# KumarRobotics/AllocNet

Hardware: AMD Instinct MI355X
Metric: MINCO trajectories solved/sec (8-seg min-snap) (higher is better)
Workload: dtype f64; 1 GPU; configs[1] problem (8-segment order-4 MINCO, random-walk waypoints, energy-only, PVA boundary c=3) at saturating batch 1048576/GPU; batch_per_gpu=1048576, row_stride_ld=1049152, pieces=8, order=4, global_batch=1048576, parallelism=dp1, ranks_seen=1, allgather_bytes_per_rank=0, allgather_every=1

## Files before the change

allocnet_amd/csrc/qp_ipm.h:

```cpp
#pragma once
#include <hip/hip_runtime.h>
#include <stdint.h>

#include <type_traits>

#include "minco_core.h"
#include "wave_ops.h"
#include "qp_admm.h"
#include "workspace_constants.h"
#include "qp_control_points.h"

namespace anet {

struct IpmArgs {
  const double *state;
  const double *T;
  const double *hpolys;
  double *sl, *lam;
  double *coeffs;
  double *obj;
  int *status, *iters;
  double *res;
  double *gradT;
  const double *grad_z;
  double *vjpT;
  int64_t B;
  int N, R, M;
  double vmax, amax, m34, tol;
  int max_iter;
  double tol_accept;
  double tol_tenth;
  int twist_min_pieces;
  const int *order;
  int it_stop, resume;
  double *cont;
  const double *tab;
#ifdef ANET_IPM_PROF
  long long *prof;
#endif
};
#ifdef ANET_IPM_PROF
#define IPM_TICK(slot)                                                          \
  do {                                                                          \
    __syncthreads();                                                            \
    if (a.prof && blockIdx.x == 0 && threadIdx.x == 0) {                        \
      const long long now_ = __builtin_readcyclecounter();                      \
      a.prof[slot] += now_ - prof_t_;                                           \
      prof_t_ = now_;                                                           \
    }                                                                           \
  } while (0)
#else
#define IPM_TICK(slot) do {} while (0)
#endif

struct IpmCorridorRow {
  double c0, c1, c2;
  static constexpr int dsel = 0;
  __device__ __forceinline__ double dot(const double (&v)[3]) const { return c0 * v[0] + c1 * v[1] + c2 * v[2]; }
  __device__ __forceinline__ void axpy(double t, double *g) const { g[0] += t * c0; g[1] += t * c1; g[2] += t * c2; }
  __device__ __forceinline__ void weights(double w, double *A) const {
    A[0] += w * c0 * c0; A[1] += w * c0 * c1; A[2] += w * c0 * c2;
    A[3] += w * c1 * c1; A[4] += w * c1 * c2; A[5] += w * c2 * c2;
  }
};
struct IpmBoxRow {
  int ax, dsel;
  double sgn;
  __device__ __forceinline__ double dot(const double (&v)[3]) const { return sgn * v[ax]; }
  __device__ __forceinline__ void axpy(double t, double *g) const { g[ax] += sgn * t; }
  __device__ __forceinline__ void weights(double w, double *A) const { A[3 + dsel * 3 + ax] += w; }
};

__host__ __device__ constexpr int ipm_ht_stride(int D) { return 3 * D + 1; }
constexpr int kIpmRecord = 31;

template <int S>
inline size_t qp_ipm_lds_bytes(int N, int R, int M) {
  constexpr int D = 2 * S, NB = 3 * D, BK = 3 * S;
  const size_t NS = (size_t)N * R;
  return sizeof(double) * ((size_t)(N + 1) * BK * 5 + (size_t)(N + 1) * BK * BK + (size_t)N * BK * BK + 3 * (size_t)N * NB +
                           (size_t)R * ipm_ht_stride(D) + 2 * D * D + (size_t)N * D + NS * kIpmRecord + (size_t)N * M * 4 + 2 * N + 32);
}

template <int S>
__global__ void __launch_bounds__(256) k_qp_ipm_tables(double *out, int R, double m34, int control_points) {
  constexpr int D = 2 * S, HS = ipm_ht_stride(D);
  const int tid = threadIdx.x, nt = blockDim.x;
  __shared__ double E[2 * D * D], Hm[D * D];
  double *Hobj = out + D * D, *ht = out + 2 * D * D;
  if (tid == 0) {
    constexpr int W = 2 * D;
    for (int r = 0; r < D; ++r)
      for (int col = 0; col < D; ++col) {
        const int d = r % S, k = D - 1 - col;
        double v = 0.0;
        if (k >= d) v = (r < S) ? (k == d ? fallf(k, d) : 0.0) : fallf(k, d);
        E[r * W + col] = v;
        E[r * W + D + col] = (r == col) ? 1.0 : 0.0;
      }
    for (int c = 0; c < D; ++c) {
      int pv = c;
      for (int r = c + 1; r < D; ++r)
        if (fabs(E[r * W + c]) > fabs(E[pv * W + c])) pv = r;
      for (int k = 0; k < W; ++k) { const double t = E[c * W + k]; E[c * W + k] = E[pv * W + k]; E[pv * W + k] = t; }
      const double ip = 1.0 / E[c * W + c];
      for (int k = 0; k < W; ++k) E[c * W + k] *= ip;
      for (int r = 0; r < D; ++r)
        if (r != c) {
          const double f = E[r * W + c];
          if (f != 0.0)
            for (int k = 0; k < W; ++k) E[r * W + k] -= f * E[c * W + k];
        }
    }
    for (int r = 0; r < D; ++r)
      for (int c = 0; c < D; ++c) Hm[r * D + c] = E[r * W + D + c];
  }
  __syncthreads();
  if (control_points) {
    const int K = R / D;
    for (int e = tid; e < K * 3 * D; e += nt) {
      const int q = e / (3 * D), d = (e / D) % 3, m = e % D;
      double c[D], beta[D];
      for (int k = 0; k < D; ++k) c[k] = Hm[(D - 1 - k) * D + m];
      qp_control_values<D>(c, d, q, K, beta);
      for (int r = 0; r < D; ++r) ht[(size_t)(q * D + r) * HS + d * D + m] = beta[r];
    }
  }
  const int n_sampled = control_points ? 0 : R * 3 * D;
  for (int e = tid; e < n_sampled; e += nt) {
    const int j = e / (3 * D), d = (e / D) % 3, m = e % D;
    const double tau = (double)j / (double)R;
    double v = 0.0;
    for (int col = 0; col < D; ++col) {
      const int k = D - 1 - col;
      if (k >= d) {
        double bv = fallf(k, d);
        for (int q = 0; q < k - d; ++q) bv *= tau;
        v += bv * Hm[col * D + m];
      }
    }
    ht[(size_t)j * HS + d * D + m] = v;
  }
  for (int e = tid; e < D * D; e += nt) {
    const int m = e / D, m2 = e % D;
    double v = 0.0;
    for (int c1 = 0; c1 < S; ++c1)
      for (int c2 = 0; c2 < S; ++c2) v += Hm[c1 * D + m] * qblk1<S>(c1, c2, m34) * Hm[c2 * D + m2];
    Hobj[e] = v;
  }
  for (int e = tid; e < D * D; e += nt) out[e] = Hm[e];
}

template <int S, int MINB = 1, bool FUSE = (MINB == 1)>
__global__ void __launch_bounds__(256, MINB) k_qp_ipm(IpmArgs a) {
  constexpr int D = 2 * S, NB = 3 * D, BK = 3 * S;
  constexpr int HS = ipm_ht_stride(D), AS = kIpmRecord;
  const int N = a.N, R = a.R, M = a.M;
  const int NS = N * R, RPS = M + 12;
  const int64_t mtot = (int64_t)NS * RPS;
  const int64_t b = a.order ? (int64_t)a.order[blockIdx.x] : (int64_t)blockIdx.x;
  const int tid = threadIdx.x, nt = blockDim.x;
  const int NY = (N + 1) * BK;
  const bool resume = a.resume != 0;
  if ((uint64_t)b >= (uint64_t)a.B) return;
  if (resume && a.status[b] != 0) return;
  double *ct = a.cont ? a.cont + b * (int64_t)(NY + kIpmContScalars) : nullptr;

#ifdef ANET_IPM_PROF
  const long long prof_start_ = __builtin_readcyclecounter();
#endif
  extern __shared__ double lds[];
  double *yv = lds;
  double *dya = yv + NY;
  double *dyc = dya + NY;
  double *rhs = dyc + NY;
  double *Dg = rhs + NY;
  double *Of = Dg + (size_t)(N + 1) * BK * BK;
  double *uu = Of + (size_t)N * BK * BK;
  double *dua = uu + (size_t)N * NB;
  double *duc = dua + (size_t)N * NB;
  double *ht = duc + (size_t)N * NB;
  double *Hobj = ht + (size_t)R * HS;
  double *Hm = Hobj + D * D;
  double *sc = Hm + D * D;
  double *acc = sc + (size_t)N * D;
  double *hp_l = acc + (size_t)NS * AS;
  double *Tn = hp_l + (size_t)N * M * 4;
  double *red = Tn + N;
  double *qsv = red + 32;
  double *dinvd = qsv + N;

  const double *Tg = a.T + b * N;
  const double *hp = a.hpolys + b * (int64_t)N * M * 4;
  const double *st = a.state + b * 18;
  double *slg = a.sl + b * mtot, *lmg = a.lam + b * mtot;

  for (int e = tid; e < N * M * 4; e += nt) hp_l[e] = hp[e];
  for (int i = tid; i < N; i += nt) {
    Tn[i] = Tg[i];
    qsv[i] = pow(Tg[i], (double)(1 - 2 * S));
  }
  {
    const double *tb = a.tab;
    for (int e = tid; e < D * D; e += nt) {
      Hm[e] = tb[e];
      Hobj[e] = tb[D * D + e];
    }
    for (int e = tid; e < R * HS; e += nt) ht[e] = tb[2 * D * D + e];
  }
  __syncthreads();
  for (int e = tid; e < N * D; e += nt) {
    const int i = e / D, m = e % D;
    double v = 1.0;
    if (m >= S && i < N - 1) v = pow(Tn[i] / Tn[i + 1], (double)(m - S));
    sc[e] = v;
  }
  for (int e = tid; e < NY; e += nt) {
    const int k = e / BK, ax = (e / S) % 3, d = e % S;
    double v = 0.0;
    if (k == 0 && d < 3) v = st[ax * 3 + d] * pow(Tn[0], (double)d);
    else if (k == N && d < 3) v = st[9 + ax * 3 + d] * pow(Tn[N - 1], (double)d);
    else if (d == 0) {
      double tsum = 0.0, tk = 0.0;
      for (int i = 0; i < N; ++i) { tsum += Tn[i]; if (i < k) tk += Tn[i]; }
      const double f = tk / tsum;
      v = (1.0 - f) * st[ax * 3] + f * st[9 + ax * 3];
    }
    yv[e] = resume ? ct[e] : v;
    dya[e] = 0.0;
    dyc[e] = 0.0;
  }
  __syncthreads();
  auto uni = [](double v) {
    return __hiloint2double(__builtin_amdgcn_readfirstlane(__double2hiint(v)), __builtin_amdgcn_readfirstlane(__double2loint(v)));
  };
  auto pinned = [&](int k, int d) { return (k == 0 || k == N) && d < 3; };
  auto fresh_tid = [&]() {
    int t = tid;
    asm volatile("" : "+v"(t));
    return t;
  };
  auto to_u = [&](const double *y, double *u) {
    for (int e = fresh_tid(); e < N * NB; e += nt) {
      const int i = e / NB, ax = (e % NB) / D, m = e % D;
      u[e] = (m < S) ? y[i * BK + ax * S + m] : sc[i * D + m] * y[(i + 1) * BK + ax * S + (m - S)];
    }
  };
  to_u(yv, uu);
  __syncthreads();

  auto state_of = [&](const double *u, int i, int j, double (&s3)[3][3]) {
    const double *hj = ht + (size_t)j * HS, *ui = u + (size_t)i * NB;
#pragma unroll
    for (int d = 0; d < 3; ++d)
#pragma unroll
      for (int ax = 0; ax < 3; ++ax) {
        double v = 0.0;
        for (int m = 0; m < D; ++m) v += hj[d * D + m] * ui[ax * D + m];
        s3[d][ax] = v;
      }
  };
  auto for_rows = [&](int i, auto &&fn) {
    for (int q = 0; q < M; ++q) {
      const double *hq = hp_l + ((size_t)i * M + q) * 4;
      const double c0 = hq[0], c1 = hq[1], c2 = hq[2];
      if (c0 == 0.0 && c1 == 0.0 && c2 == 0.0) continue;
      fn(q, IpmCorridorRow{c0, c1, c2}, hq[3]);
    }
    const double hvv = a.vmax * Tn[i], hva = a.amax * Tn[i] * Tn[i];
#pragma unroll
    for (int qq = 0; qq < 12; ++qq) {
      const int axsel = qq / 4, w4 = qq % 4, dsel = 1 + (w4 & 1);
      const double sgn = (w4 < 2) ? 1.0 : -1.0;
      fn(M + qq, IpmBoxRow{axsel, dsel, sgn}, dsel == 1 ? hvv : hva);
    }
  };
  auto for_rows_sl = [&](int i, int smp, auto store_tag, auto &&fn) {
    constexpr bool STORE = decltype(store_tag)::value;
    double *sp = slg + smp, *lp = lmg + smp;
    constexpr int GC = (STORE && FUSE) ? 4 : 8, GB = (STORE && FUSE) ? 4 : 6;
    for (int q0 = 0; q0 < M; q0 += GC) {
      double sl[GC], lm[GC];
#pragma unroll
      for (int g = 0; g < GC; ++g) {
        const int q = q0 + g < M ? q0 + g : M - 1;
        sl[g] = sp[(int64_t)q * NS];
        lm[g] = lp[(int64_t)q * NS];
      }
#pragma unroll
      for (int g = 0; g < GC; ++g) {
        const int q = q0 + g;
        if (q >= M) break;
        const double *hq = hp_l + ((size_t)i * M + q) * 4;
        const double c0 = hq[0], c1 = hq[1], c2 = hq[2];
        if (c0 == 0.0 && c1 == 0.0 && c2 == 0.0) continue;
        fn(q, IpmCorridorRow{c0, c1, c2}, hq[3], sl[g], lm[g]);
        if (STORE) {
          sp[(int64_t)q * NS] = sl[g];
          lp[(int64_t)q * NS] = lm[g];
        }
      }
    }
    const double hvv = a.vmax * Tn[i], hva = a.amax * Tn[i] * Tn[i];
#pragma unroll
    for (int g0 = 0; g0 < 12; g0 += GB) {
      double sl[GB], lm[GB];
#pragma unroll
      for (int g = 0; g < GB; ++g) {
        sl[g] = sp[(int64_t)(M + g0 + g) * NS];
        lm[g] = lp[(int64_t)(M + g0 + g) * NS];
      }
#pragma unroll
      for (int g = 0; g < GB; ++g) {
        const int qq = g0 + g, axsel = qq / 4, w4 = qq % 4, dsel = 1 + (w4 & 1);
        const double sgn = (w4 < 2) ? 1.0 : -1.0;
        fn(M + qq, IpmBoxRow{axsel, dsel, sgn}, dsel == 1 ? hvv : hva, sl[g], lm[g]);
        if (STORE) {
          sp[(int64_t)(M + qq) * NS] = sl[g];
          lp[(int64_t)(M + qq) * NS] = lm[g];
        }
      }
    }
  };
  using RowsLoad = std::integral_constant<bool, false>;
  using RowsUpdate = std::integral_constant<bool, true>;
  auto sum_index = [](int slot) { return slot == 0 ? 0 : (slot == 4 ? 1 : (slot == 5 ? 2 : 3)); };
  auto block_reduce = [&](double v, int slot, bool is_min) {
    v = is_min ? wave_min_f64(v) : wave_sum<63>(v);
    if ((tid & 63) == 0) {
      if (is_min) atomic_max_pos(&red[slot], 1.0 / fmax(v, 1e-300));
      else red[16 + 4 * sum_index(slot) + (tid >> 6)] = v;
    }
  };
  auto red_sum = [&](int slot) {
    const double *p4 = red + 16 + 4 * sum_index(slot);
    return (p4[0] + p4[1]) + (p4[2] + p4[3]);
  };

#ifndef ANET_IPM_LAM0_SCALE
#define ANET_IPM_LAM0_SCALE 1e-6
#endif
  auto first_iterate = [&]() -> double {
  if (tid < 32) red[tid] = 0.0;
  __syncthreads();
  {
    double l_p = 0.0;
    for (int e = tid; e < NY; e += nt) {
      const int k = e / BK, ax = (e / S) % 3, d = e % S;
      if (pinned(k, d)) continue;
      double vp = 0.0;
      for (int side = 0; side < 2; ++side) {
        const int i = side == 0 ? k : k - 1;
        if (i < 0 || i >= N) continue;
        const int m = side == 0 ? d : S + d;
        const double *ui = uu + (size_t)i * NB + ax * D;
        double g = 0.0;
        for (int m2 = 0; m2 < D; ++m2) g += Hobj[m * D + m2] * ui[m2];
        vp += sc[i * D + m] * qsv[i] * g;
      }
      l_p = fmax(l_p, fabs(vp));
    }
    block_reduce(1.0 / fmax(l_p, 1e-300), 3, true);
  }
  __syncthreads();
  const double lam0 = uni(fmax(1.0, ANET_IPM_LAM0_SCALE * red[3]));
  __syncthreads();
  int64_t nrows_local = 0;
  for (int smp = fresh_tid(); smp < NS; smp += nt) {
    const int i = smp / R, j = smp % R;
    double s3[3][3];
    state_of(uu, i, j, s3);
    for (int q = 0; q < RPS; ++q) {
      slg[smp + (int64_t)q * NS] = 1.0;
      lmg[smp + (int64_t)q * NS] = 0.0;
    }
    for_rows(i, [&](int q, auto row, double hv) {
      const double gy = row.dot(s3[row.dsel]);
      slg[smp + (int64_t)q * NS] = fmax(hv - gy, 1.0);
      lmg[smp + (int64_t)q * NS] = lam0;
      ++nrows_local;
    });
  }
  if (tid < 32) red[tid] = 0.0;
  __syncthreads();
  block_reduce((double)nrows_local, 0, false);
  __syncthreads();
  const double mr = uni(fmax(red_sum(0), 1.0));
  __syncthreads();
  return mr;
  };
  const double mrows = resume ? uni(ct[NY]) : first_iterate();

  auto node_vector = [&](double *out, int goff, bool with_obj, const double *u, int goff2 = -1, double w2 = 0.0, double sgn = 1.0) {
    for (int e2 = fresh_tid(); e2 < 2 * ((NY + 127) / 128) * 128; e2 += nt) {
      const int e = e2 >> 1, side = e2 & 1;
      const bool live = e < NY;
      const int k = live ? e / BK : 0, ax = (e / S) % 3, d = e % S;
      double v = 0.0;
      const int i = side == 0 ? k : k - 1;
      if (live && !pinned(k, d) && i >= 0 && i < N) {
        const int m = side == 0 ? d : S + d;
        double g = 0.0;
        if (with_obj) {
          const double qs = qsv[i];
          const double *ui = u + (size_t)i * NB + ax * D;
          for (int m2 = 0; m2 < D; ++m2) g += qs * Hobj[m * D + m2] * ui[m2];
        }
        if (goff2 < 0) {
          for (int j = 0; j < R; ++j) {
            const double *ga = acc + (size_t)(i * R + j) * AS + goff;
            const double *hj = ht + (size_t)j * HS;
            g += ga[ax] * hj[m] + ga[3 + ax] * hj[D + m] + ga[6 + ax] * hj[2 * D + m];
          }
        } else {
          for (int j = 0; j < R; ++j) {
            const double *ga = acc + (size_t)(i * R + j) * AS + goff, *gb = acc + (size_t)(i * R + j) * AS + goff2;
            const double *hj = ht + (size_t)j * HS;
            g += (ga[ax] + w2 * gb[ax]) * hj[m] + (ga[3 + ax] + w2 * gb[3 + ax]) * hj[D + m] +
                 (ga[6 + ax] + w2 * gb[6 + ax]) * hj[2 * D + m];
          }
        }
        v = sc[i * D + m] * g;
      }
      v = pair_sum(v);
      if (live && side == 0) out[e] = sgn * v;
    }
  };

  auto side_vectors = [&]() {
    const int t2 = fresh_tid() - 128;
    double l_rd = 0.0, l_py = 0.0, l_obj = 0.0;
    for (int e = t2; e < NY; e += 128) {
      const int k = e / BK, ax = (e / S) % 3, d = e % S;
      double vp = 0.0, vr = 0.0, va = 0.0;
      for (int side = 0; side < 2; ++side) {
        const int i = side == 0 ? k : k - 1;
        if (i < 0 || i >= N) continue;
        const int m = side == 0 ? d : S + d;
        const double qs = qsv[i];
        const double *ui = uu + (size_t)i * NB + ax * D;
        double g = 0.0;
        for (int m2 = 0; m2 < D; ++m2) g += qs * Hobj[m * D + m2] * ui[m2];
        double gr = g, ga = g;
        for (int j = 0; j < R; ++j) {
          const double *ac = acc + (size_t)(i * R + j) * AS;
          const double *hj = ht + (size_t)j * HS;
          gr += ac[21 + ax] * hj[m] + ac[24 + ax] * hj[D + m] + ac[27 + ax] * hj[2 * D + m];
          ga += ac[12 + ax] * hj[m] + ac[15 + ax] * hj[D + m] + ac[18 + ax] * hj[2 * D + m];
        }
        const double scm = sc[i * D + m];
        vp += scm * g;
        vr += scm * gr;
        va += scm * ga;
      }
      const bool pin = pinned(k, d);
      l_rd = fmax(l_rd, pin ? 0.0 : fabs(vr));
      l_py = fmax(l_py, fabs(vp));
      dya[e] = -(pin ? 0.0 : va);
    }
    for (int e = t2; e < N * NB; e += 128) {
      const int i = e / NB, ax = (e % NB) / D, m = e % D;
      const double *ui = uu + (size_t)i * NB + ax * D;
      double g = 0.0;
      for (int m2 = 0; m2 < D; ++m2) g += Hobj[m * D + m2] * ui[m2];
      l_obj += qsv[i] * ui[m] * g;
    }
    block_reduce(1.0 / fmax(l_rd, 1e-300), 8, true);
    block_reduce(1.0 / fmax(l_py, 1e-300), 9, true);
    block_reduce(l_obj, 10, false);
  };

  auto rl = [](double v, int lane) {
    return __hiloint2double(__builtin_amdgcn_readlane(__double2hiint(v), lane), __builtin_amdgcn_readlane(__double2loint(v), lane));
  };
  const int PT = N >= a.twist_min_pieces ? N / 2 : N;
  auto chol_rows = [&](const int lane, double (&Dr)[BK], double (&dinv)[BK]) {
#pragma unroll
    for (int c = 0; c < BK; ++c) {
      const double dcc = fmax(rl(Dr[c], c), 1e-300);
      double rs = __builtin_amdgcn_rsq(dcc);
      rs = rs * __builtin_fma(-0.5 * dcc * rs, rs, 1.5);
      rs = rs * __builtin_fma(-0.5 * dcc * rs, rs, 1.5);
      dinv[c] = rs;
      const double piv = dcc * rs;
      Dr[c] = (lane == c) ? piv : Dr[c] * dinv[c];
#pragma unroll
      for (int c2 = c + 1; c2 < BK; ++c2) Dr[c2] -= Dr[c] * rl(Dr[c], c2);
    }
  };
  typedef double d4_t __attribute__((ext_vector_type(4)));
  auto schur_mfma = [&](const int lane, const double *X, double *Dk) {
    const int li = lane & 15, lk = lane >> 4;
    d4_t c4 = {0.0, 0.0, 0.0, 0.0};
#pragma unroll
    for (int ks = 0; ks < (BK + 3) / 4; ++ks) {
      const int k = 4 * ks + lk;
      const double x = (li < BK && k < BK) ? X[li * BK + k] : 0.0;
      c4 = __builtin_amdgcn_mfma_f64_16x16x4f64(x, x, c4, 0, 0, 0);
    }
#pragma unroll
    for (int r = 0; r < 4; ++r) {
      const int row = lk + 4 * r;
      if (row < BK && li < BK) Dk[row * BK + li] -= c4[r];
    }
  };
  auto twisted_factor = [&](auto &&side) {
    const int wv = __builtin_amdgcn_readfirstlane(tid >> 6);
    int lane = tid & 63;
    asm volatile("" : "+v"(lane));
    const bool act = lane < BK;
    const int dir = wv == 0 ? 1 : -1, kfrom = wv == 0 ? 0 : N;
#pragma nounroll
    for (int ph = 0; ph < 2; ++ph) {
      if (ph == 1) __syncthreads();
      if (wv >= 2) {
        if (ph == 0) side();
        continue;
      }
      if (ph == 1 && wv == 1) continue;
      const int kbeg = ph == 0 ? kfrom : PT, kend = ph == 0 ? PT : PT + 1;
      const int stepk = ph == 0 ? dir : 1;
#pragma nounroll
      for (int k = kbeg; k != kend; k += stepk) {
        double *Dk = Dg + (size_t)k * BK * BK;
        double Dr[BK], dinv[BK];
        const int src0 = ph == 0 ? (k == kfrom ? -1 : (dir > 0 ? k - 1 : k)) : (PT > 0 ? PT - 1 : -1);
        const int src1 = ph == 0 ? -1 : (PT < N ? PT : -1);
#pragma nounroll
        for (int u = 0; u < 2; ++u) {
          const int src = u == 0 ? src0 : src1;
          if (src < 0) continue;
          schur_mfma(lane, Of + (size_t)src * BK * BK, Dk);
        }
#pragma unroll
        for (int c = 0; c < BK; ++c) Dr[c] = act ? Dk[lane * BK + c] : (c == 0 ? 1.0 : 0.0);
        chol_rows(lane, Dr, dinv);
#ifndef ANET_IPM_INV_FROM_LDS
#define ANET_IPM_INV_FROM_LDS 1
#endif
        if constexpr (ANET_IPM_INV_FROM_LDS != 0) {
          if (act) {
#pragma unroll
            for (int c = 0; c < BK; ++c) Dk[lane * BK + c] = Dr[c];
          }
        }
        double pcol[BK];
#pragma unroll
        for (int c = 0; c < BK; ++c) pcol[c] = (c == lane) ? 1.0 : 0.0;
#pragma unroll
        for (int q = 0; q < BK; ++q) {
          pcol[q] *= dinv[q];
#pragma unroll
          for (int c = q + 1; c < BK; ++c) {
            if constexpr (ANET_IPM_INV_FROM_LDS != 0) pcol[c] -= Dk[c * BK + q] * pcol[q];
            else pcol[c] -= rl(Dr[q], c) * pcol[q];
          }
        }
        if (act) {
#pragma unroll
          for (int c = 0; c < BK; ++c) Dk[c * BK + lane] = pcol[c];
        }
        if (ph == 1) continue;
        double *Lo = Of + (size_t)(dir > 0 ? k : k - 1) * BK * BK;
        const int st_c = dir > 0 ? 1 : BK, st_l = dir > 0 ? BK : 1;
        {
          const int li = lane & 15, lk = lane >> 4;
          d4_t c4 = {0.0, 0.0, 0.0, 0.0};
#pragma unroll
          for (int ks = 0; ks < (BK + 3) / 4; ++ks) {
            const int kk = 4 * ks + lk;
            const bool in = li < BK && kk < BK;
            const double av = in ? Lo[li * st_l + kk * st_c] : 0.0;
            const double bv = in ? Dk[li * BK + kk] : 0.0;
            c4 = __builtin_amdgcn_mfma_f64_16x16x4f64(av, bv, c4, 0, 0, 0);
          }
#pragma unroll
          for (int r = 0; r < 4; ++r) {
            const int row = lk + 4 * r;
            if (row < BK && li < BK) Lo[row * BK + li] = c4[r];
          }
        }
      }
    }
  };
  auto twisted_solve = [&](double *x) {
    const int wv = __builtin_amdgcn_readfirstlane(tid >> 6);
    int lane = tid & 63;
    asm volatile("" : "+v"(lane));
    const bool act = lane < BK;
    const int lr = act ? lane : 0;
    const int dir = wv == 0 ? 1 : -1, kfrom = wv == 0 ? 0 : N;
    auto matvec = [&](const double (&Mrow)[BK], const double v) {
      double acc = 0.0;
#pragma unroll
      for (int c = 0; c < BK; ++c) acc = __builtin_fma(Mrow[c], rl(v, c), acc);
      return acc;
    };
    auto load_row = [&](const double *blk, double (&dst)[BK]) {
#pragma unroll
      for (int c = 0; c < BK; ++c) dst[c] = blk[lr * BK + c];
    };
    auto load_col = [&](const double *blk, double (&dst)[BK]) {
#pragma unroll
      for (int c = 0; c < BK; ++c) dst[c] = blk[c * BK + lr];
    };
    double zmid = 0.0;
    double zprev = 0.0;
    if (wv < 2 && kfrom != PT) {
      double Lr[BK], Xr[BK], Ln[BK], Xn[BK];
      load_row(Dg + (size_t)kfrom * BK * BK, Lr);
#pragma unroll
      for (int c = 0; c < BK; ++c) Xr[c] = 0.0;
      double xin = act ? x[kfrom * BK + lane] : 0.0;
#pragma nounroll
      for (int k = kfrom; k != PT; k += dir) {
        const int kn = k + dir;
        const bool more = kn != PT;
        double xnext = 0.0;
        if (more) {
          load_row(Dg + (size_t)kn * BK * BK, Ln);
          load_row(Of + (size_t)(dir > 0 ? kn - 1 : kn) * BK * BK, Xn);
          xnext = act ? x[kn * BK + lane] : 0.0;
        }
        const double xr = xin - matvec(Xr, zprev);
        const double z = matvec(Lr, xr);
        if (act) x[k * BK + lane] = z;
        zprev = z;
        if (more) {
#pragma unroll
          for (int c = 0; c < BK; ++c) {
            Lr[c] = Ln[c];
            Xr[c] = Xn[c];
          }
          xin = xnext;
        }
      }
    }
    __syncthreads();
    if (wv == 0) {
      double Lr[BK], Xr[BK];
      double xr = act ? x[PT * BK + lane] : 0.0;
      if (PT > 0) {
        load_row(Of + (size_t)(PT - 1) * BK * BK, Xr);
        xr -= matvec(Xr, zprev);
      }
      if (PT < N) {
        load_row(Of + (size_t)PT * BK * BK, Xr);
        const double zo = act ? x[(PT + 1) * BK + lane] : 0.0;
        xr -= matvec(Xr, zo);
      }
      load_row(Dg + (size_t)PT * BK * BK, Lr);
      const double z = matvec(Lr, xr);
      load_col(Dg + (size_t)PT * BK * BK, Lr);
      zmid = matvec(Lr, z);
      if (act) x[PT * BK + lane] = zmid;
    }
    __syncthreads();
    if (wv < 2 && kfrom != PT) {
      double Lc[BK], Xc[BK], Ln[BK], Xn[BK];
      const int k0 = PT - dir;
      double xnb = wv == 0 ? zmid : (act ? x[PT * BK + lane] : 0.0);
      load_col(Dg + (size_t)k0 * BK * BK, Lc);
      load_col(Of + (size_t)(dir > 0 ? k0 : k0 - 1) * BK * BK, Xc);
      double zin = act ? x[k0 * BK + lane] : 0.0;
#pragma nounroll
      for (int k = k0; k != kfrom - dir; k -= dir) {
        const int kn = k - dir;
        const bool more = kn != kfrom - dir;
        double znext = 0.0;
        if (more) {
          load_col(Dg + (size_t)kn * BK * BK, Ln);
          load_col(Of + (size_t)(dir > 0 ? kn : kn - 1) * BK * BK, Xn);
          znext = act ? x[kn * BK + lane] : 0.0;
        }
        const double xr = zin - matvec(Xc, xnb);
        const double xo = matvec(Lc, xr);
        if (act) x[k * BK + lane] = xo;
        xnb = xo;
        if (more) {
#pragma unroll
          for (int c = 0; c < BK; ++c) {
            Lc[c] = Ln[c];
            Xc[c] = Xn[c];
          }
          zin = znext;
        }
      }
    }
  };

  auto assemble_newton = [&]() {
    for (int e = fresh_tid(); e < (2 * N + 1) * BK * BK; e += nt) Dg[e] = 0.0;
    __syncthreads();
    for (int w = fresh_tid(); w < N * D * D; w += nt) {
      const int i = w / (D * D), m = (w / D) % D, m2 = w % D;
      if (m < S && m2 >= S) continue;
      double Sa[6] = {0, 0, 0, 0, 0, 0}, Sd[3] = {0, 0, 0};
      for (int j = 0; j < R; ++j) {
        const double *as = acc + (size_t)(i * R + j) * AS;
        const double *hj = ht + (size_t)j * HS;
        const double p0 = hj[m] * hj[m2], p1 = hj[D + m] * hj[D + m2], p2 = hj[2 * D + m] * hj[2 * D + m2];
#pragma unroll
        for (int q = 0; q < 6; ++q) Sa[q] += as[q] * p0;
#pragma unroll
        for (int ax = 0; ax < 3; ++ax) Sd[ax] += as[6 + ax] * p1 + as[9 + ax] * p2;
      }
      const double scale = sc[i * D + m] * sc[i * D + m2], ob = qsv[i] * Hobj[m * D + m2];
#pragma unroll
      for (int axr = 0; axr < 3; ++axr)
#pragma unroll
        for (int axc = 0; axc < 3; ++axc) {
          const int wa = axr <= axc ? (axr == 0 ? axc : (axr == 1 ? 2 + axc : 5)) : (axc == 0 ? axr : (axc == 1 ? 2 + axr : 5));
          const double v = scale * (Sa[wa] + (axr == axc ? Sd[axr] + ob : 0.0));
          if (m < S) atomicAdd(&Dg[(size_t)i * BK * BK + (axr * S + m) * BK + axc * S + m2], v);
          else if (m2 >= S) atomicAdd(&Dg[(size_t)(i + 1) * BK * BK + (axr * S + m - S) * BK + axc * S + (m2 - S)], v);
          else Of[(size_t)i * BK * BK + (axr * S + m - S) * BK + axc * S + m2] = v;
        }
    }
    __syncthreads();
    for (int e = fresh_tid(); e < (2 * N + 1) * BK * BK; e += nt) {
      const int blk = e / (BK * BK), r = (e % (BK * BK)) / BK, c = e % BK;
      const bool diag = blk <= N;
      const int k = diag ? blk : blk - (N + 1);
      const int kr = diag ? k : k + 1, kc = k;
      double v = Dg[e];
      if (pinned(kr, r % S) || pinned(kc, c % S)) v = (diag && r == c) ? 1.0 : 0.0;
      if (diag && r == c) v += 1e-13 * fabs(v) + 1e-300;
      Dg[e] = v;
    }
  };

  int it = 0, status = -2, accepted_steps = 0;
  double pres = 0.0, dres = 0.0, mu = 0.0, mu0 = 0.0, pres_mark = INFINITY, mu_mark = INFINITY, alpha_win = 0.0;
  int stalled_windows = 0;
  double objn_last = 0.0, alpha_last = 1.0;
  bool stopped = false;
  if (resume) {
    it = (int)ct[NY + 1];
    accepted_steps = (int)ct[NY + 2];
    stalled_windows = (int)ct[NY + 3];
    mu0 = ct[NY + 4];
    pres_mark = ct[NY + 5];
    mu_mark = ct[NY + 6];
    alpha_win = ct[NY + 7];
    it = __builtin_amdgcn_readfirstlane(it);
  }
  const int it_first = it;
#ifdef ANET_IPM_PROF
  long long prof_t_ = __builtin_readcyclecounter();
  if (a.prof && blockIdx.x == 0 && threadIdx.x == 0) a.prof[13] = prof_t_ - prof_start_;
#endif
  IPM_TICK(0);
  auto row_A = [&](auto row, double hv, double gy, double sl, double lm, double *A_, double &l_mu, double &l_pres, double &l_h) {
    const double rg = gy + sl - hv, w = lm * fast_rcp1(sl), t = lm + w * (gy - hv);
    l_mu += sl * lm;
    l_pres = fmax(l_pres, fabs(rg));
    l_h = fmax(l_h, fabs(hv));
    row.weights(w, A_);
    row.axpy(t, A_ + 12 + row.dsel * 3);
    row.axpy(lm, A_ + 21 + row.dsel * 3);
  };
  auto pass_A = [&]() {
    double l_mu = 0.0, l_pres = 0.0, l_h = 0.0;
    for (int smp = fresh_tid(); smp < NS; smp += nt) {
      const int i = smp / R, j = smp % R;
      double s3[3][3];
      state_of(uu, i, j, s3);
      double A_[30];
#pragma unroll
      for (int q = 0; q < 30; ++q) A_[q] = 0.0;
      for_rows_sl(i, smp, RowsLoad{}, [&](int q, auto row, double hv, double sl, double lm) {
        row_A(row, hv, row.dot(s3[row.dsel]), sl, lm, A_, l_mu, l_pres, l_h);
      });
      double *as = acc + (size_t)smp * AS;
#pragma unroll
      for (int q = 0; q < 30; ++q) as[q] = A_[q];
    }
    block_reduce(l_mu, 0, false);
    block_reduce(1.0 / fmax(l_pres, 1e-300), 1, true);
    block_reduce(1.0 / fmax(l_h, 1e-300), 2, true);
  };
#ifndef ANET_IPM_CERT_EPS
#define ANET_IPM_CERT_EPS 1e-3
#endif
  auto certified_infeasible = [&]() -> bool {
    __syncthreads();
    if (tid < 32) red[tid] = 0.0;
    __syncthreads();
    node_vector(dya, 21, false, uu);
    double l_lh = 0.0, l_lam = 0.0;
    for (int smp = fresh_tid(); smp < NS; smp += nt) {
      const int i = smp / R, j = smp % R;
      double s3[3][3];
      state_of(uu, i, j, s3);
      for_rows_sl(i, smp, RowsLoad{}, [&](int q, auto row, double hv, double sl, double lm) {
        (void)q; (void)sl;
        l_lh += lm * (hv - row.dot(s3[row.dsel]));
        l_lam = fmax(l_lam, lm);
      });
    }
    __syncthreads();
    double l_g = 0.0, l_y = 0.0;
    for (int e = fresh_tid(); e < NY; e += nt) {
      const int k = e / BK, d = e % S;
      l_g = fmax(l_g, fabs(dya[e]));
      if (!pinned(k, d)) l_y += dya[e] * yv[e];
    }
    block_reduce(l_lh, 0, false);
    block_reduce(l_y, 4, false);
    block_reduce(1.0 / fmax(l_lam, 1e-300), 1, true);
    block_reduce(1.0 / fmax(l_g, 1e-300), 2, true);
    __syncthreads();
    const double lh = uni(red_sum(0)) + uni(red_sum(4)), lam_max = uni(red[1]), g_max = uni(red[2]);
    __syncthreads();
    if (tid < 32) red[tid] = 0.0;
    __syncthreads();
#ifdef ANET_IPM_CERT_TRACE
    if (tid == 0) printf("ipm cert problem %lld it %d: lh/lam %.3e g/lam %.3e\n", (long long)b, it, lh / lam_max, g_max / lam_max);
#endif
    return g_max <= ANET_IPM_CERT_EPS * lam_max && lh <= -ANET_IPM_CERT_EPS * lam_max;
  };
  if (tid < 32) red[tid] = 0.0;
  __syncthreads();
  if constexpr (FUSE) {
    pass_A();
    __syncthreads();
  }
  for (it = it_first; it < a.max_iter; ++it) {
    if (a.it_stop > 0 && it == a.it_stop && !resume) {
      stopped = true;
      break;
    }
    if constexpr (!FUSE) {
      if (tid < 32) red[tid] = 0.0;
      __syncthreads();
      double l_mu = 0.0, l_pres = 0.0, l_h = 0.0;
      for (int smp = fresh_tid(); smp < NS; smp += nt) {
        const int i = smp / R, j = smp % R;
        double s3[3][3];
        state_of(uu, i, j, s3);
        double A_[30];
#pragma unroll
        for (int q = 0; q < 30; ++q) A_[q] = 0.0;
        for_rows_sl(i, smp, RowsLoad{}, [&](int q, auto row, double hv, double sl, double lm) {
          const double gy = row.dot(s3[row.dsel]);
          const double rg = gy + sl - hv, w = lm * fast_rcp1(sl), t = lm + w * (gy - hv);
          l_mu += sl * lm;
          l_pres = fmax(l_pres, fabs(rg));
          l_h = fmax(l_h, fabs(hv));
          row.weights(w, A_);
          row.axpy(t, A_ + 12 + row.dsel * 3);
          row.axpy(lm, A_ + 21 + row.dsel * 3);
        });
        double *as = acc + (size_t)smp * AS;
#pragma unroll
        for (int q = 0; q < 30; ++q) as[q] = A_[q];
      }
      block_reduce(l_mu, 0, false);
      block_reduce(1.0 / fmax(l_pres, 1e-300), 1, true);
      block_reduce(1.0 / fmax(l_h, 1e-300), 2, true);
      __syncthreads();
    }
    IPM_TICK(1);
    mu = uni(red_sum(0) / mrows);
    if (it == 0) mu0 = mu;
    pres = uni(red[1] / fmax(1.0, red[2]));
    __syncthreads();
    if constexpr (FUSE)
      if (tid < 32) red[tid] = 0.0;
    assemble_newton();
    __syncthreads();
    IPM_TICK(3);
    twisted_factor(side_vectors);
    __syncthreads();
    IPM_TICK(5);
    dres = uni(red[8] / fmax(1.0, red[9]));
    const double objn = uni(red_sum(10));
    objn_last = objn;
    if (pres < a.tol && dres < a.tol && mu * mrows < a.tol * fmax(1.0, 0.5 * fabs(objn))) { status = 1; break; }
    if (a.tol_accept > a.tol && pres < a.tol_accept && dres < a.tol_accept &&
        mu * mrows < a.tol_accept * fmax(1.0, 0.5 * fabs(objn)) && ++accepted_steps > 8) { status = 1; break; }
    if (!(mu == mu) || mu > 1e12 * fmax(mu0, 1.0)) { status = -3; break; }
#ifdef ANET_IPM_TRACE
    if (tid == 0 && blockIdx.x == ANET_IPM_TRACE && it % 5 == 0)
      printf("ipm trace it %d pres %.3e dres %.3e mu %.3e alpha_win %.3f obj %.6e\n", it, pres, dres, mu, alpha_win, objn);
#endif
#ifndef ANET_IPM_GROWTH_PRES
#define ANET_IPM_GROWTH_PRES 0.5
#endif
    if (it % 10 == 0) {
      const bool shortsteps = it >= 20 && alpha_win < 0.5;
      const bool growth = shortsteps && pres > a.tol && pres > ANET_IPM_GROWTH_PRES * pres_mark && mu > 1.2 * mu_mark;
      const bool stall = shortsteps && pres > 1e-4 && pres > 0.7 * pres_mark && mu > 0.5 * mu_mark;
      stalled_windows = (growth || stall) ? stalled_windows + 1 : 0;
      if (stalled_windows >= 2 && certified_infeasible()) { status = -3; break; }
      pres_mark = pres;
      mu_mark = mu;
      alpha_win = 0.0;
    }
    twisted_solve(dya);
    __syncthreads();
    IPM_TICK(6);
    to_u(dya, dua);
    if (tid < 32) red[tid] = 0.0;
    __syncthreads();
    {
      double l_ap = 0.0, l_s1 = 0.0, l_s2 = 0.0;
      for (int smp = fresh_tid(); smp < NS; smp += nt) {
        const int i = smp / R, j = smp % R;
        double s3[3][3], d3[3][3], G0[9], G1[9];
        state_of(uu, i, j, s3);
        state_of(dua, i, j, d3);
#pragma unroll
        for (int q = 0; q < 9; ++q) G0[q] = G1[q] = 0.0;
        for_rows_sl(i, smp, RowsLoad{}, [&](int q, auto row, double hv, double sl, double lm) {
          const double rg = row.dot(s3[row.dsel]) + sl - hv;
          const double ds = -rg - row.dot(d3[row.dsel]);
          const double isl = fast_rcp1(sl);
          const double dl = -lm - (lm * isl) * ds;
          l_ap = fmax(l_ap, fmax(-ds * isl, -dl * __builtin_amdgcn_rcp(lm)));
          l_s1 += sl * dl + lm * ds;
          l_s2 += ds * dl;
          const double t0 = lm + (lm * rg - sl * lm - ds * dl) * isl;
          row.axpy(t0, G0 + row.dsel * 3);
          row.axpy(isl, G1 + row.dsel * 3);
        });
        double *as = acc + (size_t)smp * AS;
#pragma unroll
        for (int q = 0; q < 9; ++q) {
          as[12 + q] = G0[q];
          as[q] = G1[q];
        }
      }
      block_reduce(1.0 / fmax(l_ap, 1e-300), 3, true);
      block_reduce(l_s1, 4, false);
      block_reduce(l_s2, 5, false);
    }
    __syncthreads();
    IPM_TICK(7);
    const double a_aff = fmin(1.0, red[3] > 0.0 ? 1.0 / red[3] : 1.0);
    const double mu_aff = uni((mu * mrows + a_aff * red_sum(4) + a_aff * a_aff * red_sum(5)) / mrows);
    double sigma = mu_aff / mu;
    sigma = sigma * sigma * sigma;
    const double mu_target = uni(fmax(sigma * mu, a.tol_tenth * fmax(1.0, 0.5 * fabs(objn)) / mrows));
    node_vector(dyc, 12, true, uu, 0, mu_target, -1.0);
    __syncthreads();
    IPM_TICK(9);
    twisted_solve(dyc);
    __syncthreads();
    IPM_TICK(10);
    to_u(dyc, duc);
    if (tid < 32) red[tid] = 0.0;
    __syncthreads();
    auto final_dir = [&](auto row, double hv, const double (&s3)[3][3], const double (&d3)[3][3],
                         const double (&e3)[3][3], double sl, double lm, double &ds, double &dl) {
      const double rg = row.dot(s3[row.dsel]) + sl - hv;
      const double dsa = -rg - row.dot(d3[row.dsel]);
      const double isl = fast_rcp1(sl);
      const double dla = -lm - (lm * isl) * dsa;
      const double rc = sl * lm + dsa * dla - mu_target;
      ds = -rg - row.dot(e3[row.dsel]);
      dl = (-rc - lm * ds) * isl;
    };
    {
      double l_a = 0.0;
      for (int smp = fresh_tid(); smp < NS; smp += nt) {
        const int i = smp / R, j = smp % R;
        double s3[3][3], d3[3][3], e3[3][3];
        state_of(uu, i, j, s3);
        state_of(dua, i, j, d3);
        state_of(duc, i, j, e3);
        for_rows_sl(i, smp, RowsLoad{}, [&](int q, auto row, double hv, double sl, double lm) {
          double ds, dl;
          final_dir(row, hv, s3, d3, e3, sl, lm, ds, dl);
          l_a = fmax(l_a, fmax(-ds * __builtin_amdgcn_rcp(sl), -dl * __builtin_amdgcn_rcp(lm)));
        });
      }
      block_reduce(1.0 / fmax(l_a, 1e-300), 6, true);
    }
    __syncthreads();
    IPM_TICK(11);
#ifndef ANET_IPM_STEP_FRACTION
#define ANET_IPM_STEP_FRACTION 0.99
#endif
    constexpr double step_fraction = ANET_IPM_STEP_FRACTION;
    const double alpha = uni(fmin(1.0, step_fraction * (red[6] > 0.0 ? 1.0 / red[6] : 1e300)));
    alpha_win = uni(fmax(alpha_win, alpha));
    alpha_last = alpha;
    __syncthreads();
    if constexpr (!FUSE) {
      for (int smp = fresh_tid(); smp < NS; smp += nt) {
        const int i = smp / R, j = smp % R;
        double s3[3][3], d3[3][3], e3[3][3];
        state_of(uu, i, j, s3);
        state_of(dua, i, j, d3);
        state_of(duc, i, j, e3);
        for_rows_sl(i, smp, RowsUpdate{}, [&](int q, auto row, double hv, double &sl, double &lm) {
          double ds, dl;
          final_dir(row, hv, s3, d3, e3, sl, lm, ds, dl);
          sl += alpha * ds;
          lm += alpha * dl;
        });
      }
    } else
    {
      double l_mu = 0.0, l_pres = 0.0, l_h = 0.0;
      for (int smp = fresh_tid(); smp < NS; smp += nt) {
        const int i = smp / R, j = smp % R;
        double s3[3][3], d3[3][3], e3[3][3];
        state_of(uu, i, j, s3);
        state_of(dua, i, j, d3);
        state_of(duc, i, j, e3);
        double A_[30];
#pragma unroll
        for (int q = 0; q < 30; ++q) A_[q] = 0.0;
        for_rows_sl(i, smp, RowsUpdate{}, [&](int q, auto row, double hv, double &sl, double &lm) {
          const double gy = row.dot(s3[row.dsel]), ge = row.dot(e3[row.dsel]);
          const double rg = gy + sl - hv;
          const double dsa = -rg - row.dot(d3[row.dsel]);
          const double isl = fast_rcp1(sl);
          const double dla = -lm - (lm * isl) * dsa;
          const double rc = sl * lm + dsa * dla - mu_target;
          const double ds = -rg - ge;
          const double dl = (-rc - lm * ds) * isl;
          sl += alpha * ds;
          lm += alpha * dl;
          row_A(row, hv, gy + alpha * ge, sl, lm, A_, l_mu, l_pres, l_h);
        });
        double *as = acc + (size_t)smp * AS;
#pragma unroll
        for (int q = 0; q < 30; ++q) as[q] = A_[q];
      }
      block_reduce(l_mu, 0, false);
      block_reduce(1.0 / fmax(l_pres, 1e-300), 1, true);
      block_reduce(1.0 / fmax(l_h, 1e-300), 2, true);
    }
    __syncthreads();
    for (int e = fresh_tid(); e < NY; e += nt) yv[e] += alpha * dyc[e];
    __syncthreads();
    to_u(yv, uu);
    __syncthreads();
    IPM_TICK(12);
  }
  __syncthreads();
  if (stopped) {
    for (int e = fresh_tid(); e < NY; e += nt) ct[e] = yv[e];
    if (tid == 0) {
      ct[NY] = mrows;
      ct[NY + 1] = (double)it;
      ct[NY + 2] = (double)accepted_steps;
      ct[NY + 3] = (double)stalled_windows;
      ct[NY + 4] = mu0;
      ct[NY + 5] = pres_mark;
      ct[NY + 6] = mu_mark;
      ct[NY + 7] = alpha_win;
      ct[NY + 8] = pres;
      ct[NY + 9] = dres;
      ct[NY + 10] = mu * mrows / fmax(1.0, 0.5 * fabs(objn_last));
      ct[NY + 11] = alpha_last;
      a.status[b] = 0;
      a.iters[b] = it;
    }
    return;
  }
  if (a.grad_z && a.vjpT) {
    const double *gz = a.grad_z + b * (int64_t)N * NB;
    double pmax = 0.0;
    for (int i = 0; i < N; ++i)
      for (int m = 0; m < D; ++m) pmax = fmax(pmax, qsv[i] * Hobj[m * D + m] * sc[i * D + m] * sc[i * D + m]);
    const double w_act = 1.0e4 * pmax;
    for (int smp = fresh_tid(); smp < NS; smp += nt) {
      const int i = smp / R;
      double A_[12];
#pragma unroll
      for (int q = 0; q < 12; ++q) A_[q] = 0.0;
      for_rows_sl(i, smp, RowsLoad{}, [&](int q, auto row, double, double sl, double lm) {
        row.weights((lm > sl) ? w_act : 0.0, A_);
      });
      double *as = acc + (size_t)smp * AS;
#pragma unroll
      for (int q = 0; q < 12; ++q) as[q] = A_[q];
    }
    __syncthreads();
    assemble_newton();
    __syncthreads();
    twisted_factor([] {});
    for (int e = fresh_tid(); e < N * NB; e += nt) {
      const int i = e / NB, ax = (e % NB) / D, m = e % D;
      double v = 0.0, tk = 1.0;
      const double rT = 1.0 / Tn[i];
      for (int col = D - 1; col >= 0; --col) {
        v += gz[(size_t)i * NB + ax * D + col] * tk * Hm[col * D + m];
        tk *= rT;
      }
      duc[e] = v;
    }
    __syncthreads();
    for (int e = fresh_tid(); e < NY; e += nt) {
      const int k = e / BK, ax = (e / S) % 3, d = e % S;
      double v = 0.0;
      if (!pinned(k, d)) {
        if (k < N) v += sc[k * D + d] * duc[(size_t)k * NB + ax * D + d];
        if (k > 0) v += sc[(k - 1) * D + S + d] * duc[(size_t)(k - 1) * NB + ax * D + S + d];
      }
      dyc[e] = v;
    }
    for (int i = fresh_tid(); i < 3 * N; i += nt) rhs[i] = 0.0;
    for (int smp = fresh_tid(); smp < NS; smp += nt) {
      double *as = acc + (size_t)smp * AS + 12;
#pragma unroll
      for (int q = 0; q < 9; ++q) as[q] = 0.0;
      as[-12] = 0.0;
      as[-11] = 0.0;
    }
    __syncthreads();
    for (int pass = 0; pass < 4; ++pass) {
      node_vector(dya, 12, false, uu);
      __syncthreads();
      for (int e = fresh_tid(); e < NY; e += nt) dya[e] = -dyc[e] - dya[e];
      __syncthreads();
      twisted_solve(dya);
      __syncthreads();
      to_u(dya, dua);
      __syncthreads();
      for (int smp = fresh_tid(); smp < NS; smp += nt) {
        const int i = smp / R, j = smp % R;
        double d3[3][3], G_[9], bsv = 0.0, bsa = 0.0;
        state_of(dua, i, j, d3);
#pragma unroll
        for (int q = 0; q < 9; ++q) G_[q] = 0.0;
        for_rows_sl(i, smp, RowsLoad{}, [&](int q, auto row, double, double sl, double lm) {
          const double dl = ((lm > sl) ? w_act : 0.0) * row.dot(d3[row.dsel]);
          row.axpy(dl, G_ + row.dsel * 3);
          if (row.dsel == 1) bsv += dl;
          if (row.dsel == 2) bsa += dl;
        });
        double *as = acc + (size_t)smp * AS + 12;
#pragma unroll
        for (int q = 0; q < 9; ++q) as[q] += G_[q];
        as[-12] += bsv;
        as[-11] += bsa;
      }
      __syncthreads();
    }
    for (int i = fresh_tid(); i < N; i += nt) {
      double sv = 0.0, sa = 0.0;
      for (int j = 0; j < R; ++j) {
        sv += acc[(size_t)(i * R + j) * AS];
        sa += acc[(size_t)(i * R + j) * AS + 1];
      }
      rhs[N + i] = sv;
      rhs[2 * N + i] = sa;
    }
    double *cA = Dg, *cB = Dg + (size_t)N * NB;
    for (int e = fresh_tid(); e < N * NB; e += nt) {
      const int i = e / NB, ax = (e % NB) / D, m = e % D, d = m % S;
      const double *ui = uu + (size_t)i * NB + ax * D, *vi = dua + (size_t)i * NB + ax * D;
      double hu = 0.0, hv = 0.0;
      for (int m2 = 0; m2 < D; ++m2) {
        hu += Hobj[m * D + m2] * ui[m2];
        hv += Hobj[m * D + m2] * vi[m2];
      }
      double t = (double)(1 - 2 * S) * qsv[i] * ui[m] * hv / Tn[i];
      {
        const int col = m, k = D - 1 - col;
        double cc = 0.0;
        for (int m2 = 0; m2 < D; ++m2) cc += Hm[col * D + m2] * ui[m2];
        t -= (double)k * cc * pow(Tn[i], (double)(-k)) * gz[(size_t)i * NB + ax * D + col] / Tn[i];
      }
      cA[e] = t;
      cB[e] = 0.0;
      if (d == 0) continue;
      double g = qsv[i] * hu, dg = qsv[i] * hv;
      for (int j = 0; j < R; ++j) {
        const double *ga = acc + (size_t)(i * R + j) * AS;
        const double *hj = ht + (size_t)j * HS;
        g += ga[21 + ax] * hj[m] + ga[24 + ax] * hj[D + m] + ga[27 + ax] * hj[2 * D + m];
        dg += ga[12 + ax] * hj[m] + ga[15 + ax] * hj[D + m] + ga[18 + ax] * hj[2 * D + m];
      }
      const double c = (dg * ui[m] + g * vi[m] + duc[e] * ui[m]) * (double)d;
      if (m >= S) {
        if (i < N - 1) {
          cA[e] = t + c / Tn[i];
          cB[e] = -c / Tn[i + 1];
        } else if (d < 3) {
          cA[e] = t + c / Tn[i];
        }
      } else if (i == 0 && d < 3) {
        cA[e] = t + c / Tn[0];
      }
    }
    __syncthreads();
    for (int i = fresh_tid(); i < N; i += nt) {
      double r = 0.0;
      for (int q = 0; q < NB; ++q) r += cA[i * NB + q];
      if (i > 0)
        for (int q = 0; q < NB; ++q) r += cB[(i - 1) * NB + q];
      a.vjpT[b * N + i] = r - (a.vmax * rhs[N + i] + 2.0 * a.amax * Tn[i] * rhs[2 * N + i]);
    }
    __syncthreads();
  }
  if (a.gradT) {
    double *cA = Dg, *cB = Dg + (size_t)N * NB;
    for (int e = fresh_tid(); e < N * NB; e += nt) {
      const int i = e / NB, ax = (e % NB) / D, m = e % D, d = m % S;
      const double *ui = uu + (size_t)i * NB + ax * D;
      double hu = 0.0;
      for (int m2 = 0; m2 < D; ++m2) hu += Hobj[m * D + m2] * ui[m2];
      const double t = (double)(1 - 2 * S) * 0.5 * qsv[i] * ui[m] * hu / Tn[i];
      cA[e] = t;
      cB[e] = 0.0;
      if (d == 0) continue;
      double g = qsv[i] * hu;
      for (int j = 0; j < R; ++j) {
        const double *ga = acc + (size_t)(i * R + j) * AS + 21;
        const double *hj = ht + (size_t)j * HS;
        g += ga[ax] * hj[m] + ga[3 + ax] * hj[D + m] + ga[6 + ax] * hj[2 * D + m];
      }
      const double c = g * ui[m] * (double)d;
      if (m >= S) {
        if (i < N - 1) {
          cA[e] = t + c / Tn[i];
          cB[e] = -c / Tn[i + 1];
        } else if (d < 3) {
          cA[e] = t + c / Tn[i];
        }
      } else if (i == 0 && d < 3) {
        cA[e] = t + c / Tn[0];
      }
    }
    for (int smp = fresh_tid(); smp < NS; smp += nt) {
      const int i = smp / R;
      double sv = 0.0, sa = 0.0;
      for (int qq = 0; qq < 12; ++qq) {
        const double lm = lmg[smp + (int64_t)(M + qq) * NS];
        if ((qq % 4) & 1) sa += lm;
        else sv += lm;
      }
      acc[(size_t)smp * AS + 30] = -(a.vmax * sv + 2.0 * a.amax * Tn[i] * sa);
    }
    __syncthreads();
    for (int i = fresh_tid(); i < N; i += nt) {
      double r = 0.0;
      for (int q = 0; q < NB; ++q) r += cA[i * NB + q];
      if (i > 0)
        for (int q = 0; q < NB; ++q) r += cB[(i - 1) * NB + q];
      for (int j = 0; j < R; ++j) r += acc[(size_t)(i * R + j) * AS + 30];
      a.gradT[b * N + i] = r;
    }
    __syncthreads();
  }
  for (int e = fresh_tid(); e < N * NB; e += nt) {
    const int i = e / NB, ax = (e % NB) / D, col = e % D, k = D - 1 - col;
    const double *ui = uu + (size_t)i * NB + ax * D;
    double v = 0.0;
    for (int m = 0; m < D; ++m) v += Hm[col * D + m] * ui[m];
    a.coeffs[b * (int64_t)N * NB + e] = v * pow(Tn[i], (double)(-k));
  }
  if (tid == 0) {
    double obj = 0.0;
    for (int i = 0; i < N; ++i) {
      const double qs = qsv[i];
      for (int ax = 0; ax < 3; ++ax) {
        const double *ui = uu + (size_t)i * NB + ax * D;
        for (int m = 0; m < D; ++m)
          for (int m2 = 0; m2 < D; ++m2) obj += 0.5 * qs * ui[m] * Hobj[m * D + m2] * ui[m2];
      }
    }
    a.obj[b] = obj;
    a.status[b] = status;
    a.iters[b] = it;
    a.res[b * 2] = pres;
    a.res[b * 2 + 1] = dres;
  }
}

int launch_qp_ipm_fuse(int s, int64_t batch, size_t lds_bytes, hipStream_t st, const IpmArgs &a);

}
```

Baseline: 2.605 billion trajectories/s.

## Compact live corridor rows into a packed per-segment slack/dual layout

Compacts non-degenerate corridor half-planes to the front of each segment's list in LDS and records the live count and a per-segment prefix offset. The slack and dual arrays are re-indexed into a packed layout (segment block plus row times R), so loops run only over live rows and skip the zero-row checks and the padded slots. This trims loads, stores and branches in the hot row loops, at the cost of a prefix-offset table and 32-bit byte addressing. External code that reads sl/lam in the old [q*NS] layout, such as resume or warm start, could become inconsistent.

```diff
diff --git a/allocnet_amd/csrc/qp_ipm.h b/allocnet_amd/csrc/qp_ipm.h
--- a/allocnet_amd/csrc/qp_ipm.h
+++ b/allocnet_amd/csrc/qp_ipm.h
@@ -78,8 +78,10 @@
 inline size_t qp_ipm_lds_bytes(int N, int R, int M) {
   constexpr int D = 2 * S, NB = 3 * D, BK = 3 * S;
   const size_t NS = (size_t)N * R;
+  const size_t row_index = ((size_t)N * 2 * sizeof(int) + sizeof(double) - 1) / sizeof(double);
   return sizeof(double) * ((size_t)(N + 1) * BK * 5 + (size_t)(N + 1) * BK * BK + (size_t)N * BK * BK + 3 * (size_t)N * NB +
-                           (size_t)R * ipm_ht_stride(D) + 2 * D * D + (size_t)N * D + NS * kIpmRecord + (size_t)N * M * 4 + 2 * N + 32);
+                           (size_t)R * ipm_ht_stride(D) + 2 * D * D + (size_t)N * D + NS * kIpmRecord + (size_t)N * M * 4 + 2 * N + 32 +
+                           row_index);
 }
 
 template <int S>
@@ -189,6 +191,8 @@
   double *red = Tn + N;
   double *qsv = red + 32;
   double *dinvd = qsv + N;
+  int *blk = (int *)(dinvd + NY);
+  int *liv = blk + N;
 
   const double *Tg = a.T + b * N;
   const double *hp = a.hpolys + b * (int64_t)N * M * 4;
@@ -209,6 +213,18 @@
     for (int e = tid; e < R * HS; e += nt) ht[e] = tb[2 * D * D + e];
   }
   __syncthreads();
+  for (int i = tid; i < N; i += nt) {
+    int L = 0;
+    for (int q = 0; q < M; ++q) {
+      const double *hq = hp_l + ((size_t)i * M + q) * 4;
+      const double c0 = hq[0], c1 = hq[1], c2 = hq[2], c3 = hq[3];
+      if (c0 == 0.0 && c1 == 0.0 && c2 == 0.0) continue;
+      double *hr = hp_l + ((size_t)i * M + L) * 4;
+      hr[0] = c0; hr[1] = c1; hr[2] = c2; hr[3] = c3;
+      ++L;
+    }
+    liv[i] = L;
+  }
   for (int e = tid; e < N * D; e += nt) {
     const int i = e / D, m = e % D;
     double v = 1.0;
@@ -231,6 +247,11 @@
     dyc[e] = 0.0;
   }
   __syncthreads();
+  for (int i = tid; i < N; i += nt) {
+    int rows = 0;
+    for (int i2 = 0; i2 < i; ++i2) rows += liv[i2] + 12;
+    blk[i] = rows * R;
+  }
   auto uni = [](double v) {
     return __hiloint2double(__builtin_amdgcn_readfirstlane(__double2hiint(v)), __builtin_amdgcn_readfirstlane(__double2loint(v)));
   };
@@ -261,63 +282,66 @@
       }
   };
   auto for_rows = [&](int i, auto &&fn) {
-    for (int q = 0; q < M; ++q) {
-      const double *hq = hp_l + ((size_t)i * M + q) * 4;
-      const double c0 = hq[0], c1 = hq[1], c2 = hq[2];
-      if (c0 == 0.0 && c1 == 0.0 && c2 == 0.0) continue;
-      fn(q, IpmCorridorRow{c0, c1, c2}, hq[3]);
+    const int L = liv[i];
+    for (int r = 0; r < L; ++r) {
+      const double *hq = hp_l + ((size_t)i * M + r) * 4;
+      fn(r, IpmCorridorRow{hq[0], hq[1], hq[2]}, hq[3]);
     }
     const double hvv = a.vmax * Tn[i], hva = a.amax * Tn[i] * Tn[i];
 #pragma unroll
     for (int qq = 0; qq < 12; ++qq) {
       const int axsel = qq / 4, w4 = qq % 4, dsel = 1 + (w4 & 1);
       const double sgn = (w4 < 2) ? 1.0 : -1.0;
-      fn(M + qq, IpmBoxRow{axsel, dsel, sgn}, dsel == 1 ? hvv : hva);
-    }
-  };
+      fn(L + qq, IpmBoxRow{axsel, dsel, sgn}, dsel == 1 ? hvv : hva);
+    }
+  };
+  const unsigned row_step = (unsigned)R * (unsigned)sizeof(double);
+  auto row_at = [&](int i, int j, int r) { return (unsigned)(blk[i] + j) * (unsigned)sizeof(double) + (unsigned)r * row_step; };
+  auto rs_load = [](const double *slot, unsigned at) { return *(const double *)((const char *)slot + at); };
+  auto rs_store = [](double *slot, unsigned at, double v) { *(double *)((char *)slot + at) = v; };
   auto for_rows_sl = [&](int i, int smp, auto store_tag, auto &&fn) {
     constexpr bool STORE = decltype(store_tag)::value;
-    double *sp = slg + smp, *lp = lmg + smp;
+    const int L = liv[i];
+    const unsigned at0 = row_at(i, smp - i * R, 0);
     constexpr int GC = (STORE && FUSE) ? 4 : 8, GB = (STORE && FUSE) ? 4 : 6;
-    for (int q0 = 0; q0 < M; q0 += GC) {
+    for (int r0 = 0; r0 < L; r0 += GC) {
       double sl[GC], lm[GC];
 #pragma unroll
       for (int g = 0; g < GC; ++g) {
-        const int q = q0 + g < M ? q0 + g : M - 1;
-        sl[g] = sp[(int64_t)q * NS];
-        lm[g] = lp[(int64_t)q * NS];
+        const int r = r0 + g < L ? r0 + g : L - 1;
+        sl[g] = rs_load(slg, at0 + (unsigned)r * row_step);
+        lm[g] = rs_load(lmg, at0 + (unsigned)r * row_step);
       }
 #pragma unroll
       for (int g = 0; g < GC; ++g) {
-        const int q = q0 + g;
-        if (q >= M) break;
-        const double *hq = hp_l + ((size_t)i * M + q) * 4;
-        const double c0 = hq[0], c1 = hq[1], c2 = hq[2];
-        if (c0 == 0.0 && c1 == 0.0 && c2 == 0.0) continue;
-        fn(q, IpmCorridorRow{c0, c1, c2}, hq[3], sl[g], lm[g]);
+        const int r = r0 + g;
+        if (r >= L) break;
+        const double *hq = hp_l + ((size_t)i * M + r) * 4;
+        fn(r, IpmCorridorRow{hq[0], hq[1], hq[2]}, hq[3], sl[g], lm[g]);
         if (STORE) {
-          sp[(int64_t)q * NS] = sl[g];
-          lp[(int64_t)q * NS] = lm[g];
+          rs_store(slg, at0 + (unsigned)r * row_step, sl[g]);
+          rs_store(lmg, at0 + (unsigned)r * row_step, lm[g]);
         }
       }
     }
     const double hvv = a.vmax * Tn[i], hva = a.amax * Tn[i] * Tn[i];
+    const unsigned atb = at0 + (unsigned)L * row_step;
 #pragma unroll
     for (int g0 = 0; g0 < 12; g0 += GB) {
       double sl[GB], lm[GB];
 #pragma unroll
       for (int g = 0; g < GB; ++g) {
-        sl[g] = sp[(int64_t)(M + g0 + g) * NS];
-        lm[g] = lp[(int64_t)(M + g0 + g) * NS];
+        sl[g] = rs_load(slg, atb + (unsigned)(g0 + g) * row_step);
+        lm[g] = rs_load(lmg, atb + (unsigned)(g0 + g) * row_step);
       }
 #pragma unroll
       for (int g = 0; g < GB; ++g) {
         const int qq = g0 + g, axsel = qq / 4, w4 = qq % 4, dsel = 1 + (w4 & 1);
         const double sgn = (w4 < 2) ? 1.0 : -1.0;
-        fn(M + qq, IpmBoxRow{axsel, dsel, sgn}, dsel == 1 ? hvv : hva, sl[g], lm[g]);
+        fn(L + qq, IpmBoxRow{axsel, dsel, sgn}, dsel == 1 ? hvv : hva, sl[g], lm[g]);
         if (STORE) {
-          sp[(int64_t)(M + qq) * NS] = sl[g];
-          lp[(int64_t)(M + qq) * NS] = lm[g];
+          rs_store(slg, atb + (unsigned)qq * row_step, sl[g]);
+          rs_store(lmg, atb + (unsigned)qq * row_step, lm[g]);
         }
       }
     }
@@ -370,14 +394,11 @@
     const int i = smp / R, j = smp % R;
     double s3[3][3];
     state_of(uu, i, j, s3);
-    for (int q = 0; q < RPS; ++q) {
-      slg[smp + (int64_t)q * NS] = 1.0;
-      lmg[smp + (int64_t)q * NS] = 0.0;
-    }
-    for_rows(i, [&](int q, auto row, double hv) {
+    for_rows(i, [&](int r, auto row, double hv) {
       const double gy = row.dot(s3[row.dsel]);
-      slg[smp + (int64_t)q * NS] = fmax(hv - gy, 1.0);
-      lmg[smp + (int64_t)q * NS] = lam0;
+      const unsigned at = row_at(i, j, r);
+      rs_store(slg, at, fmax(hv - gy, 1.0));
+      rs_store(lmg, at, lam0);
       ++nrows_local;
     });
   }
@@ -1231,9 +1252,10 @@
     }
     for (int smp = fresh_tid(); smp < NS; smp += nt) {
       const int i = smp / R;
+      const unsigned atb = row_at(i, smp - i * R, liv[i]);
       double sv = 0.0, sa = 0.0;
       for (int qq = 0; qq < 12; ++qq) {
-        const double lm = lmg[smp + (int64_t)(M + qq) * NS];
+        const double lm = rs_load(lmg, atb + (unsigned)qq * row_step);
         if ((qq % 4) & 1) sa += lm;
         else sv += lm;
       }
```

After: 2.613 billion trajectories/s, median of 3. About the same (+0.3%).
